# linum-uqam/ViT-OCM-WMSegmentation

Hardware: AMD Instinct MI355X
Metric: OCM tiles/s (224x224, ViT-S/16 attention-map inference) (higher is better)
Workload: dtype bf16x3

## Files before the change

vit-ocm-wmsegmentation_amd/csrc/gemm_core.h:

```cpp
#pragma once
#include <type_traits>
#include "common.h"

#ifdef OCM_GEMM_STAMPS
__device__ unsigned long long g_wstamps[512 * 16 * 8];
#define WSTAMP(k)                                                                                       \
    do {                                                                                                \
        if (t == nsteps / 2 && (threadIdx.x & 63) == 0 && blockIdx.x < 512)                              \
            g_wstamps[(blockIdx.x * 16 + (threadIdx.x >> 6 & 15)) * 8 + (k)] = __builtin_readcyclecounter(); \
    } while (0)
__device__ unsigned long long g_stamps[8192 * 8];
#define STAMP(i)                                                                                        \
    do {                                                                                                \
        if (threadIdx.x == 0 && blockIdx.x < 8192) g_stamps[blockIdx.x * 8 + (i)] = __builtin_readcyclecounter(); \
    } while (0)
#else
#define STAMP(i) ((void)0)
#define WSTAMP(k) ((void)0)
#endif

template <int BM_, int BN_, int WAVES_M_, int WAVES_N_, int MF16_ = 0>
struct GemmCfg {
    static constexpr int BM = BM_, BN = BN_, WAVES_M = WAVES_M_, WAVES_N = WAVES_N_, MF16 = MF16_;
    static constexpr int NT = WAVES_M * WAVES_N * OCM_WAVE;
// ... 187 lines not shown
    for (int i = 0; i < A_CH; ++i) {
        const int q = tid + NT * i, row = q >> 3;
        a_h[i] = al.row(min(m0 + row, M - 1));
        a_off[i] = lds_off(row, cc);
    }
#pragma unroll
    for (int i = 0; i < B_CH; ++i) {
        const int q = tid + NT * i, row = q >> 3;
        b_h[i] = (const char *)W + (int64_t)min(n0 + row, N - 1) * ldw * (int)sizeof(E) + cc * 16;
        b_off[i] = lds_off(row, cc);
    }
    struct Slot {
        typename ALoad::Raw a[A_CH];
        Chunk b[B_CH];
    };
    auto issue = [&](Slot &sl, int t) {
#pragma unroll
        for (int i = 0; i < A_CH; ++i) sl.a[i] = al.load(a_h[i], t, cc);
#pragma unroll
#if defined(OCM_ABL) && (OCM_ABL == 9 || OCM_ABL == 10)
        for (int i = 0; i < B_CH; ++i) sl.b[i] = *(const Chunk *)(b_h[i]);
#else
        for (int i = 0; i < B_CH; ++i) {
            if constexpr (aload_w_tail<ALoad>::v) {
                sl.b[i] = Chunk{};
                if (t * 128 + cc * 16 < al.w_row_bytes) sl.b[i] = *(const Chunk *)(b_h[i] + t * 128);
            } else {
                sl.b[i] = *(const Chunk *)(b_h[i] + t * 128);
            }
        }
#endif
    };
    auto commit = [&](int buf, const Slot &sl) {
#pragma unroll
        for (int i = 0; i < A_CH; ++i) *(Chunk *)(As + buf * BM * 128 + a_off[i]) = ALoad::finish(sl.a[i], cc);
#pragma unroll
        for (int i = 0; i < B_CH; ++i) *(Chunk *)(Bs + buf * BN * 128 + b_off[i]) = sl.b[i];
    };
    auto compute = [&](int buf) {
        mma_step<Cfg, E, SWAP>(As + buf * BM * 128 + (wm * 32) * 128, Bs + buf * BN * 128 + (wn * 32) * 128, r, h, acc);
    };

    constexpr int ACCL = accl_of<Cfg, E>();
#pragma unroll
    for (int j = 0; j < TN; ++j) {
        const int nb = n0 + (j * Cfg::WAVES_N + wn) * 32;
#pragma unroll
        for (int e = 0; e < 16; ++e) {
            const float bv = bias ? bias[min(nb + (SWAP ? acc_rpos<ACCL>(e, lane) : acc_cpos<ACCL>(e, lane)), N - 1)] : 0.f;
#pragma unroll
            for (int i = 0; i < TM; ++i) acc[i][j][e] = bv;
        }
    }

    if constexpr (KSTEPS > 0) {
#if defined(OCM_ABL) && OCM_ABL == 11
        auto issue2 = [&](Slot &sl, int t) { if (t < 3) issue(sl, min(t, KSTEPS - 1)); };
#else
        auto issue2 = [&](Slot &sl, int t) { issue(sl, min(t, KSTEPS - 1)); };
#endif
        Slot s0, s1;
        issue2(s0, 0);
        issue2(s1, 1);
        commit(0, s0);
        issue2(s0, 2);
        lds_barrier();
#ifdef OCM_GEMM_STAMPS
        STAMP(6);
#endif
        if constexpr (KSTEPS % 2 == 0 && Elem<E>::MODE == 2 && NT == 512 && OCM_PINGPONG) {
            auto phase_barrier = [&]() {
                __builtin_amdgcn_sched_barrier(0);
                lds_barrier();
                __builtin_amdgcn_sched_barrier(0);
            };
            const int grp = __builtin_amdgcn_readfirstlane(wave >> 2);
            if (grp == 0) {
                for (int t = 0; t < KSTEPS; t += 2) {
                    compute(0);
                    phase_barrier();
                    commit(1, s1);
                    issue2(s1, t + 3);
                    phase_barrier();
                    compute(1);
                    phase_barrier();
                    commit(0, s0);
                    issue2(s0, t + 4);
                    phase_barrier();
                }
            } else {
                for (int t = 0; t < KSTEPS; t += 2) {
                    commit(1, s1);
                    issue2(s1, t + 3);
                    phase_barrier();
                    compute(0);
                    phase_barrier();
                    commit(0, s0);
                    issue2(s0, t + 4);
                    phase_barrier();
                    compute(1);
                    phase_barrier();
                }
            }
        } else if constexpr (KSTEPS % 2 == 0) {
            for (int t = 0; t < KSTEPS; t += 2) {
                compute(0);
                commit(1, s1);
                issue2(s1, t + 3);
                lds_barrier();
                compute(1);
                commit(0, s0);
                issue2(s0, t + 4);
                lds_barrier();
            }
        } else {
#pragma unroll
            for (int t = 0; t < KSTEPS; ++t) {
                compute(t & 1);
                if (t & 1) {
                    if (t + 1 < KSTEPS) commit(0, s0);
                    issue2(s0, t + 3);
                } else {
                    if (t + 1 < KSTEPS) commit(1, s1);
                    issue2(s1, t + 3);
                }
                lds_barrier();
            }
        }
    } else {
        const int nt = K / KROW;
        Slot s0;
        issue(s0, 0);
        commit(0, s0);
        lds_barrier();
        for (int t = 0; t < nt; ++t) {
            const int buf = t & 1;
            if (t + 1 < nt) issue(s0, t + 1);
            compute(buf);
            if (t + 1 < nt) commit(buf ^ 1, s0);
            lds_barrier();
        }
    }
}

#define OCM_VMCNT(n) asm volatile("s_waitcnt vmcnt(%0)" ::"n"(n) : "memory")

__device__ __forceinline__ void raw_barrier() {
    asm volatile("s_waitcnt lgkmcnt(0)" ::: "memory");
    __builtin_amdgcn_s_barrier();
    asm volatile("" ::: "memory");
}

template <int LPS, int S>
__device__ __forceinline__ void wait_vm_steps(int younger) {
    if constexpr (S == 0) {
        OCM_VMCNT(0);
    } else {
        if (younger >= S)
            OCM_VMCNT(S * LPS);
        else
            wait_vm_steps<LPS, S - 1>(younger);
    }
}

template <int CNT, int NW, int AUX = 0>
__device__ __forceinline__ void dma_rows(__amdgpu_buffer_rsrc_t rs, char *img, const int (&voff)[CNT], int wave,
                                         int soff) {
#if defined(__HIP_DEVICE_COMPILE__)
    typedef __attribute__((address_space(3))) void *lds_ptr;
#pragma unroll
    for (int j = 0; j < CNT; ++j)
        __builtin_amdgcn_raw_ptr_buffer_load_lds(rs, (lds_ptr)(img + (j * NW + wave) * 1024), 16, voff[j], soff, 0, AUX);
#endif
}

template <int CNT, int AUX = 0>
__device__ __forceinline__ void dma_pieces(__amdgpu_buffer_rsrc_t rs, char *img, const int (&voff)[CNT], const int (&piece)[CNT],
                                           int soff) {
#if defined(__HIP_DEVICE_COMPILE__)
    typedef __attribute__((address_space(3))) void *lds_ptr;
#pragma unroll
    for (int j = 0; j < CNT; ++j)
        __builtin_amdgcn_raw_ptr_buffer_load_lds(rs, (lds_ptr)(img + piece[j] * 1024), 16, voff[j], soff, 0, AUX);
#endif
}

template <class Cfg, class E, bool SWAP, int KSTEPS, int NSTAGE, int A_AUX = 0>
__device__ __forceinline__ void gemm_mainloop_dma(const E *__restrict__ A, int64_t lda, const E *__restrict__ W,
                                                  int64_t ldw, int m0, int n0, int M, int N, int K, char *smem,
                                                  f32x16 (&acc)[Cfg::TM][Cfg::TN], const float *__restrict__ bias) {
    constexpr int BM = Cfg::BM, BN = Cfg::BN, NT = Cfg::NT, NW = NT / 64;
    constexpr int TM = Cfg::TM, TN = Cfg::TN;
    constexpr int A_P = BM / 8, A_I = (A_P + NW - 1) / NW, B_I = BN / 8 / NW, LPS = A_I + B_I;
    constexpr int STAGE = (BM + BN) * 128, D = NSTAGE - 1;
    static_assert(BM % 8 == 0 && BN % (8 * NW) == 0 && (A_P % NW == 0 || 2 * (A_P % NW) >= NW), "each wave fills whole groups of 8 rows");
    static_assert(NSTAGE >= 2 && NSTAGE <= 4, "2..4 LDS stages");
    const int tid = threadIdx.x, lane = tid & 63;
    const int wave = __builtin_amdgcn_readfirstlane(tid >> 6);
    const int wm = wave / Cfg::WAVES_N, wn = wave % Cfg::WAVES_N;
    const int r = lane & 31, h = lane >> 5;
    const int esz = (int)sizeof(E);
    const int nsteps = KSTEPS > 0 ? KSTEPS : K / Elem<E>::KROW;

    auto bound = [](int64_t rows, int64_t ld_bytes) {
        const int64_t b = rows * ld_bytes;
        return (unsigned)(b > 0xFFFFFFFFll ? 0xFFFFFFFFll : b);
    };
    const auto rsA = __builtin_amdgcn_make_buffer_rsrc((void *)((const char *)A + (int64_t)m0 * lda * esz), 0,
                                                       bound(M - m0, lda * esz), 0x00020000);
    const auto rsB = __builtin_amdgcn_make_buffer_rsrc((void *)((const char *)W + (int64_t)n0 * ldw * esz), 0,
                                                       bound(N - n0, ldw * esz), 0x00020000);
    int voffA[A_I], voffB[B_I];
    int pieceA[A_I];
#pragma unroll
    for (int j = 0; j < A_I; ++j) {
        int pc = j * NW + wave;
        if (pc >= A_P) pc -= A_P % NW;
        pieceA[j] = pc;
        const int rho = pc * 8 + (lane >> 3);
        voffA[j] = rho * (int)(lda * esz) + (((lane & 7) ^ ((rho >> 1) & 7)) << 4);
    }
#pragma unroll
    for (int j = 0; j < B_I; ++j) {
        const int rho = (j * NW + wave) * 8 + (lane >> 3);
        voffB[j] = rho * (int)(ldw * esz) + (((lane & 7) ^ ((rho >> 1) & 7)) << 4);
    }
#define OCM_DMA_ISSUE(t, buf)                                                   \
    do {                                                                        \
        char *st_ = smem + (buf) * STAGE;                                       \
        dma_pieces<A_I, A_AUX>(rsA, st_, voffA, pieceA, (t) * 128);             \
        dma_rows<B_I, NW>(rsB, st_ + BM * 128, voffB, wave, (t) * 128);         \
    } while (0)
    auto compute = [&](int buf) {
        const char *st = smem + buf * STAGE;
        mma_step<Cfg, E, SWAP>(st + (wm * 32) * 128, st + BM * 128 + (wn * 32) * 128, r, h, acc, wm);
    };

    constexpr int ACCL = accl_of<Cfg, E>();
    constexpr int NBV = SWAP ? 16 : (ACCL ? 2 : 1);
    float bv[TN][NBV];
#pragma unroll
    for (int j = 0; j < TN; ++j) {
        const int nb = n0 + (j * Cfg::WAVES_N + wn) * 32;
#pragma unroll
        for (int e = 0; e < NBV; ++e)
            bv[j][e] = bias ? bias[min(nb + (SWAP ? acc_rpos<ACCL>(e, lane) : acc_cpos<ACCL>(4 * e, lane)), N - 1)] : 0.f;
    }
#pragma unroll
    for (int t = 0; t < D; ++t)
        if (t < nsteps) OCM_DMA_ISSUE(t, t);
#pragma unroll
    for (int j = 0; j < TN; ++j)
#pragma unroll
        for (int i = 0; i < TM; ++i)
#pragma unroll
            for (int e = 0; e < 16; ++e) acc[i][j][e] = bv[j][SWAP ? e : (ACCL ? ((e >> 2) & 1) : 0)];
    int bc = 0, bi = D % NSTAGE;
#ifdef OCM_GEMM_STAMPS
    unsigned long long stamp_wait = 0;
#endif
    for (int t = 0; t < nsteps; ++t) {
        const int younger = min(D - 1, nsteps - 1 - t);
#ifdef OCM_GEMM_STAMPS
        const unsigned long long tw0 = __builtin_readcyclecounter();
#endif
        WSTAMP(0);
        wait_vm_steps<LPS, NSTAGE - 2>(younger);
        WSTAMP(1);
#ifdef OCM_GEMM_STAMPS
        const unsigned long long tw1 = __builtin_readcyclecounter();
#endif
        raw_barrier();
#ifdef OCM_GEMM_STAMPS
        if (t == 0) STAMP(6);
        if (t > 0) {
            const unsigned long long tw2 = __builtin_readcyclecounter();
            stamp_wait += ((tw2 - tw1) << 32) | ((tw1 - tw0) & 0xFFFFFFFFull);
        }
#endif
        WSTAMP(2);
#if !defined(OCM_ABL) || OCM_ABL != 2
        if (t + D < nsteps) OCM_DMA_ISSUE(t + D, bi);
#endif
        __builtin_amdgcn_sched_barrier(0);
        WSTAMP(3);
        compute(bc);
#ifdef OCM_GEMM_STAMPS
        if (t == nsteps / 2) {
            __builtin_amdgcn_sched_barrier(0);
            asm volatile("v_mov_b32 %0, %0\n\ts_nop 0" : "+v"(acc[TM - 1][TN - 1][15]));
            WSTAMP(4);
        }
#endif
        bc = bc + 1 == NSTAGE ? 0 : bc + 1;
        bi = bi + 1 == NSTAGE ? 0 : bi + 1;
    }
    raw_barrier();
#ifdef OCM_GEMM_STAMPS
    if (threadIdx.x == 0 && blockIdx.x < 8192) g_stamps[blockIdx.x * 8 + 7] = stamp_wait;
#endif
#undef OCM_DMA_ISSUE
}

constexpr int EPI_MAXS = 6;
struct EpiPre {
    f32x2 raw[EPI_MAXS];
    f32x2 cd;
};
struct EpiNoPre {};
template <class Cfg, class Epi>
__device__ __forceinline__ auto epi_prefetch(const Epi &epi, int m0, int n0, int M, int N) {
    if constexpr (Epi::ROWTAB) {
        EpiPre p;
#pragma unroll
        for (int i = 0; i < EPI_MAXS; ++i) p.raw[i] = f32x2{0.f, 0.f};
        p.cd = f32x2{0.f, 0.f};
        if (threadIdx.x < Cfg::BM) epi.row_raw(min(m0 + (int)threadIdx.x, M - 1), p.raw);
        if (threadIdx.x < Cfg::BN) p.cd = epi.col_entry(min(n0 + (int)threadIdx.x, N - 1));
        return p;
    } else {
        return EpiNoPre();
    }
}

template <class Cfg, bool SWAP, class Epi, int LDS_AVAIL = Cfg::LDS_BYTES, class Pre = EpiNoPre, int ACCL = 0>
__device__ __forceinline__ void run_epilogue(const f32x16 (&acc)[Cfg::TM][Cfg::TN], char *smem, const Epi &epi, int m0,
                                             int n0, bool active = true, const Pre *pre = nullptr) {
    f32x2 *rowtab = (f32x2 *)(smem + LDS_AVAIL), *coltab = rowtab + Cfg::BM;
    if constexpr (Epi::ROWTAB) {
        if (threadIdx.x < Cfg::BM) rowtab[threadIdx.x] = epi.row_final(pre->raw);
        if (threadIdx.x < Cfg::BN) coltab[threadIdx.x] = pre->cd;
    }
    const int lane = threadIdx.x & 63, wave = threadIdx.x >> 6;
    const int wm = wave / Cfg::WAVES_N, wn = wave % Cfg::WAVES_N;
    const int r = lane & 31, h = lane >> 5;
    if constexpr (Cfg::BM * Cfg::BN * 4 <= LDS_AVAIL) {
        constexpr int COLS = SWAP ? Cfg::BM : Cfg::BN;
        float *C = (float *)smem;
        if (active)
#pragma unroll
        for (int i = 0; i < Cfg::TM; ++i)
#pragma unroll
            for (int j = 0; j < Cfg::TN; ++j) {
                const bool half = Cfg::HALF && i == Cfg::TM - 1;
                const int tm = half ? (Cfg::TM - 1) * Cfg::RB + wm * 16 : (i * Cfg::WAVES_M + wm) * 32, tn = (j * Cfg::WAVES_N + wn) * 32;
                const int row0 = SWAP ? tn : tm, col0 = SWAP ? tm : tn;
#pragma unroll
                for (int e = 0; e < (half ? 8 : 16); ++e)
                    C[(row0 + acc_rpos<ACCL>(e, lane)) * COLS + col0 + acc_cpos<ACCL>(e, lane)] = acc[i][j][e];
            }
        STAMP(2);
        lds_barrier();
        STAMP(3);
        if (active) epi.template run<PassCfg<Cfg::BM, Cfg::BN, Cfg::NT>>((const float *)C, m0, n0, rowtab, coltab);
    } else if constexpr (!SWAP) {
        constexpr int PASS = Cfg::RB * Cfg::BN * 4;
        static_assert(PASS <= LDS_AVAIL, "a row band must fit the operand LDS");
        constexpr int NBUF = 2 * PASS <= LDS_AVAIL ? 2 : 1;
#pragma unroll
        for (int i = 0; i < Cfg::TM; ++i) {
            if (NBUF == 1 && i) lds_barrier();
            float *C = (float *)(smem + (i % NBUF) * PASS);
            const bool half = Cfg::HALF && i == Cfg::TM - 1;
            if (active)
#pragma unroll
            for (int j = 0; j < Cfg::TN; ++j) {
                const int col0 = (j * Cfg::WAVES_N + wn) * 32;
#pragma unroll
                for (int e = 0; e < (half ? 8 : 16); ++e)
                    C[(wm * (half ? 16 : 32) + acc_rpos<ACCL>(e, lane)) * Cfg::BN + col0 + acc_cpos<ACCL>(e, lane)] = acc[i][j][e];
            }
            lds_barrier();
            if (active) {
                if (half)
                    epi.template run<PassCfg<Cfg::RB / 2, Cfg::BN, Cfg::NT>>((const float *)C, m0 + i * Cfg::RB, n0, rowtab + i * Cfg::RB, coltab);
                else
                    epi.template run<PassCfg<Cfg::RB, Cfg::BN, Cfg::NT>>((const float *)C, m0 + i * Cfg::RB, n0, rowtab + i * Cfg::RB, coltab);
            }
        }
    } else {
        static_assert(!Cfg::HALF, "half tiles: normal orientation only");
        constexpr int PASS = Cfg::CB * Cfg::BM * 4;
        static_assert(PASS <= LDS_AVAIL, "a column band must fit the operand LDS");
        constexpr int NBUF = 2 * PASS <= LDS_AVAIL ? 2 : 1;
#pragma unroll
        for (int j = 0; j < Cfg::TN; ++j) {
            if (NBUF == 1 && j) lds_barrier();
            float *C = (float *)(smem + (j % NBUF) * PASS);
            if (active)
#pragma unroll
            for (int i = 0; i < Cfg::TM; ++i) {
                const int col0 = (i * Cfg::WAVES_M + wm) * 32;
#pragma unroll
                for (int e = 0; e < 16; ++e)
                    C[(wn * 32 + acc_rpos<ACCL>(e, lane)) * Cfg::BM + col0 + acc_cpos<ACCL>(e, lane)] = acc[i][j][e];
            }
            lds_barrier();
            if (active) epi.template run<PassCfg<Cfg::BM, Cfg::CB, Cfg::NT>>((const float *)C, m0, n0 + j * Cfg::CB, rowtab, coltab + j * Cfg::CB);
        }
    }
}

template <class Cfg, class E, bool SWAP, int KSTEPS, int NSTAGE, class Epi, int A_AUX = 0>
__global__ __launch_bounds__(Cfg::NT) void gemm_dma_kernel(const E *__restrict__ A, int64_t lda, const E *__restrict__ W,
                                                           int64_t ldw, int M, int N, int K, Epi epi) {
    extern __shared__ __attribute__((aligned(16))) char smem[];
    const int tiles_n = (N + Cfg::BN - 1) / Cfg::BN;
    const int id = xcd_remap(blockIdx.x, gridDim.x);
    const int tm = id / tiles_n, tn = id - tm * tiles_n;
    const int m0 = tm * Cfg::BM, n0 = tn * Cfg::BN;
    f32x16 acc[Cfg::TM][Cfg::TN];
    const auto pre = epi_prefetch<Cfg>(epi, m0, n0, M, N);
    STAMP(0);
#if defined(OCM_ABL) && OCM_ABL == 4
#pragma unroll
    for (int i = 0; i < Cfg::TM; ++i)
#pragma unroll
        for (int j = 0; j < Cfg::TN; ++j)
#pragma unroll
            for (int e = 0; e < 16; ++e) acc[i][j][e] = (float)(threadIdx.x + e);
#else
    gemm_mainloop_dma<Cfg, E, SWAP, KSTEPS, NSTAGE, A_AUX>(A, lda, W, ldw, m0, n0, M, N, K, smem, acc, epi.bias);
#endif
    STAMP(1);
#if defined(OCM_ABL) && OCM_ABL == 3
#pragma unroll
    for (int i = 0; i < Cfg::TM; ++i)
#pragma unroll
        for (int j = 0; j < Cfg::TN; ++j) asm volatile("" ::"v"(acc[i][j]));
#else
    run_epilogue<Cfg, SWAP, Epi, NSTAGE * (Cfg::BM + Cfg::BN) * 128, decltype(pre), accl_of<Cfg, E>()>(acc, smem, epi, m0, n0, true, &pre);
#endif
    STAMP(4);
#ifdef OCM_GEMM_STAMPS
    __builtin_amdgcn_s_waitcnt(0);
    STAMP(5);
#endif
}

template <class Cfg, class E, bool SWAP, int KSTEPS, class ALoad, class Epi>
__global__ __launch_bounds__(Cfg::NT) void gemm_kernel(ALoad al, const E *__restrict__ W, int64_t ldw, int M, int N,
                                                       int K, Epi epi) {
    extern __shared__ __attribute__((aligned(16))) char smem[];
    const int tiles_n = (N + Cfg::BN - 1) / Cfg::BN;
    const int id = xcd_remap(blockIdx.x, gridDim.x);
    const int tm = id / tiles_n, tn = id - tm * tiles_n;
    const int m0 = tm * Cfg::BM, n0 = tn * Cfg::BN;
    f32x16 acc[Cfg::TM][Cfg::TN];
    const auto pre = epi_prefetch<Cfg>(epi, m0, n0, M, N);
    STAMP(0);
    gemm_mainloop<Cfg, E, SWAP, KSTEPS>(al, W, ldw, m0, n0, M, N, K, smem, acc, epi.bias);
    STAMP(1);
    run_epilogue<Cfg, SWAP, Epi, Cfg::LDS_BYTES, decltype(pre), accl_of<Cfg, E>()>(acc, smem, epi, m0, n0, true, &pre);
    STAMP(4);
#ifdef OCM_GEMM_STAMPS
    __builtin_amdgcn_s_waitcnt(0);
    STAMP(5);
#endif
}
```

vit-ocm-wmsegmentation_amd/csrc/gemm_kernels.h:

```cpp
#pragma once
#include <type_traits>
#include "gemm_core.h"
#include "launch.h"
#include "dev_knobs.h"

int ocm_wt_mask();

#ifndef OCM_SMALLM_STAGES
#define OCM_SMALLM_STAGES 4
#endif
constexpr int OCM_SMALLM_ROWS = 4096;
typedef GemmCfg<128, 128, 2, 2> Cfg128x128;
typedef GemmCfg<128, 128, 2, 4> Cfg128x128q;
typedef GemmCfg<128, 128, 2, 4, 1> Cfg128x128q16;
typedef GemmCfg<128, 128, 2, 2, 1> Cfg128x128m16;
typedef GemmCfg<160, 128, 2, 4, 1> Cfg160x128q16;
typedef GemmCfg<256, 256, 2, 4, 1> Cfg256x256m16;
typedef GemmCfg<64, 128, 2, 2> Cfg64x128;
typedef GemmCfg<64, 128, 2, 4> Cfg64x128w;
typedef GemmCfg<64, 64, 2, 2> Cfg64x64;
typedef GemmCfg<256, 256, 2, 4> Cfg256x256;

static inline bool big_tiles_pay(int M, int N, int K) {
    return K >= 768 && N % 256 == 0 && (long)((M + 255) / 256) * (N / 256) >= 512;
// ... 746 lines not shown
                                const float v = e < 4 ? v0[e & 3] : v1[e & 3];
                                store_act1((E *)nullptr, (char *)vt + ((int64_t)(bb * H + head) * hd + d) * npad * 4, tt, v);
                                if (qkv32) qkv32[((((int64_t)2 * B + bb) * H + head) * ntok + tt) * hd + d] = v;
                            }
                            if (++tt == ntok) {
                                tt = 0;
                                ++bb;
                            }
                        }
                    }
                }
                return;
            }
        }
        constexpr int RS = NT >= BM ? NT / BM : 1;
        static_assert(NT >= BM, "one lane per token column");
        if (threadIdx.x >= RS * BM) return;
        const int col = threadIdx.x % BM, m = m0 + col;
        if (m >= M) return;
        const int b = m / ntok, t = m - b * ntok;
        const f32x2 mr = rowtab[col];
        const float mu = mr[0], rstd = mr[1];
#pragma unroll 4
        for (int row = threadIdx.x / BM; row < BN; row += RS) {
            const int rem = rem0 + row;
            const int head = hd == 64 ? rem >> 6 : rem / hd, d = rem - head * hd;
            float v = C[row * BM + col];
            if (ln.stats) {
                const f32x2 cd = coltab[row];
                v = fmaf(rstd, fmaf(-mu, cd[0], v), cd[1]);
            }
            if (vt) store_act1((E *)nullptr, (char *)vt + ((int64_t)(b * H + head) * hd + d) * npad * (int)sizeof(E), t, v);
            if (qkv32) qkv32[((((int64_t)2 * B + b) * H + head) * ntok + t) * hd + d] = v;
        }
    }
};

template <class Cfg, class E, int KSTEPS>
__global__ __launch_bounds__(Cfg::NT) void qkv_kernel(RowLoader<E> al, const E *__restrict__ W, int M, int D,
                                                      EpiQK<E> eqk, EpiVt<E> ev) {
    extern __shared__ __attribute__((aligned(16))) char smem[];
    const int N = 3 * D, K = D;
    const int tiles_n = (ev.want_v ? N : 2 * D) / Cfg::BN;
    const int id = xcd_remap(blockIdx.x, gridDim.x);
    const int tm = id / tiles_n, tn = id - tm * tiles_n;
    const int m0 = tm * Cfg::BM, n0 = tn * Cfg::BN;
    f32x16 acc[Cfg::TM][Cfg::TN];
    const auto pre = epi_prefetch<Cfg>(eqk, m0, n0, M, N);
    if (n0 < 2 * D) {
        gemm_mainloop<Cfg, E, false, KSTEPS>(al, W, K, m0, n0, M, N, K, smem, acc, eqk.bias);
        run_epilogue<Cfg, false, EpiQK<E>, Cfg::LDS_BYTES, decltype(pre), accl_of<Cfg, E>()>(acc, smem, eqk, m0, n0, true, &pre);
    } else {
        gemm_mainloop<Cfg, E, true, KSTEPS>(al, W, K, m0, n0, M, N, K, smem, acc, ev.bias);
        run_epilogue<Cfg, true, EpiVt<E>, Cfg::LDS_BYTES, decltype(pre), accl_of<Cfg, E>()>(acc, smem, ev, m0, n0, true, &pre);
    }
}

template <class Cfg, class E, int KSTEPS, int NSTAGE>
__global__ __launch_bounds__(Cfg::NT) void qkv_dma_kernel(const E *__restrict__ A, const E *__restrict__ W, int M, int D,
                                                          EpiQK<E> eqk, EpiVt<E> ev) {
    extern __shared__ __attribute__((aligned(16))) char smem[];
    const int N = 3 * D, K = D;
    const int tiles_n = (ev.want_v ? N : 2 * D) / Cfg::BN;
    const int id = xcd_remap(blockIdx.x, gridDim.x);
    const int tm = id / tiles_n, tn = id - tm * tiles_n;
    const int m0 = tm * Cfg::BM, n0 = tn * Cfg::BN;
    f32x16 acc[Cfg::TM][Cfg::TN];
    const auto pre = epi_prefetch<Cfg>(eqk, m0, n0, M, N);
    constexpr int RING = NSTAGE * (Cfg::BM + Cfg::BN) * 128;
    if (n0 < 2 * D) {
        gemm_mainloop_dma<Cfg, E, false, KSTEPS, NSTAGE>(A, K, W, K, m0, n0, M, N, K, smem, acc, eqk.bias);
        run_epilogue<Cfg, false, EpiQK<E>, RING, decltype(pre), accl_of<Cfg, E>()>(acc, smem, eqk, m0, n0, true, &pre);
    } else {
        gemm_mainloop_dma<Cfg, E, true, KSTEPS, NSTAGE>(A, K, W, K, m0, n0, M, N, K, smem, acc, ev.bias);
        run_epilogue<Cfg, true, EpiVt<E>, RING, decltype(pre), accl_of<Cfg, E>()>(acc, smem, ev, m0, n0, true, &pre);
    }
}

template <class Cfg, class E, int KSTEPS, int NSTAGE>
static hipError_t launch_qkv_dma_ks(const E *a, const E *w, int M, int D, const EpiQK<E> &eqk, const EpiVt<E> &ev,
                                    hipStream_t s) {
    auto kern = qkv_dma_kernel<Cfg, E, KSTEPS, NSTAGE>;
    constexpr int LDS = NSTAGE * (Cfg::BM + Cfg::BN) * 128 + (Cfg::BM + Cfg::BN) * 8;
    static OptinMask optin;
    if (hipError_t e = lds_optin((const void *)kern, LDS, optin); e != hipSuccess) return e;
    const int tiles = ((M + Cfg::BM - 1) / Cfg::BM) * ((ev.want_v ? 3 : 2) * D / Cfg::BN);
    kern<<<dim3(tiles), dim3(Cfg::NT), LDS, s>>>(a, w, M, D, eqk, ev);
    return hipGetLastError();
}

template <class Cfg, class E, int NSTAGE>
static hipError_t launch_qkv_dma(const E *a, const E *w, int M, int D, const EpiQK<E> &eqk, const EpiVt<E> &ev,
                                 hipStream_t s) {
    switch (D / Elem<E>::KROW) {
        case 12: return launch_qkv_dma_ks<Cfg, E, 12, NSTAGE>(a, w, M, D, eqk, ev, s);
        case 24: return launch_qkv_dma_ks<Cfg, E, 24, NSTAGE>(a, w, M, D, eqk, ev, s);
        default: break;
    }
    return launch_qkv_dma_ks<Cfg, E, 0, NSTAGE>(a, w, M, D, eqk, ev, s);
}

template <class Cfg, class E, int KSTEPS>
static hipError_t launch_qkv_ks(const RowLoader<E> &al, const E *w, int M, int D, const EpiQK<E> &eqk,
                                const EpiVt<E> &ev, hipStream_t s) {
    auto kern = qkv_kernel<Cfg, E, KSTEPS>;
    constexpr int LDS = Cfg::LDS_BYTES + (Cfg::BM + Cfg::BN) * 8;
    static OptinMask optin;
    if (hipError_t e = lds_optin((const void *)kern, LDS, optin); e != hipSuccess) return e;
    const int tiles = ((M + Cfg::BM - 1) / Cfg::BM) * ((ev.want_v ? 3 : 2) * D / Cfg::BN);
    kern<<<dim3(tiles), dim3(Cfg::NT), LDS, s>>>(al, w, M, D, eqk, ev);
    return hipGetLastError();
}

template <class Cfg, class E>
static hipError_t launch_qkv_cfg(const RowLoader<E> &al, const E *w, int M, int D, const EpiQK<E> &eqk,
                                 const EpiVt<E> &ev, hipStream_t s) {
    switch (D / Elem<E>::KROW) {
        case 6: return launch_qkv_ks<Cfg, E, 6>(al, w, M, D, eqk, ev, s);
        case 12: return launch_qkv_ks<Cfg, E, 12>(al, w, M, D, eqk, ev, s);
        case 24: return launch_qkv_ks<Cfg, E, 24>(al, w, M, D, eqk, ev, s);
        default: break;
    }
    return launch_qkv_ks<Cfg, E, 0>(al, w, M, D, eqk, ev, s);
}

template <class E>
hipError_t launch_qkv_e(const E *a, const E *w, const float *bias, E *q, E *k, E *vt, float *qkv_f32, int batch,
                               int n_tokens, int n_pad, int heads, int head_dim, bool want_v, hipStream_t s,
                               const LnFold &ln) {
    const int D = heads * head_dim, M = batch * n_tokens;
    if (head_dim != 64 && head_dim != 128 && (q || k || vt)) return hipErrorInvalidValue;
    if (head_dim % 8) return hipErrorInvalidValue;
    if (D % 64) return hipErrorInvalidValue;
    RowLoader<E> al{a, D};
    EpiQK<E> eqk{bias, q, k, qkv_f32, M, n_tokens, n_pad, heads, D, batch, head_dim};
    eqk.wt = (ocm_wt_mask() >> 1) & 1;
    EpiVt<E> ev{bias, vt, qkv_f32, M, n_tokens, n_pad, heads, D, batch, head_dim, want_v};
    if (ln.stats) {
        eqk.ln = ev.ln = ln;
        eqk.bias = ev.bias = nullptr;
        if (OCM_KNOB(6) == 1) eqk.ln.stats = ev.ln.stats = nullptr;
        if (OCM_KNOB(6) == 2) eqk.ln.nslot = ev.ln.nslot = 1;
    }
    if constexpr (Elem<E>::MODE == 0)
        if (D % 256 == 0 && big_tiles_pay(M, 3 * D, D)) return launch_qkv_cfg<Cfg256x256, E>(al, w, M, D, eqk, ev, s);
    const long t128 = (long)((M + 127) / 128) * (3 * D / 128);
    if constexpr (Elem<E>::MODE == 2) {
        if (D % 128 == 0 && M > 64) {
#ifdef OCM_DEV
            switch (OCM_KNOB(3)) {
                case 1: return launch_qkv_dma<Cfg128x128, E, 2>(a, w, M, D, eqk, ev, s);
                case 2: return launch_qkv_dma<Cfg128x128q, E, 2>(a, w, M, D, eqk, ev, s);
                case 3: return launch_qkv_dma<Cfg64x128, E, 2>(a, w, M, D, eqk, ev, s);
                case 4: if (D % 256 == 0) return launch_qkv_dma<Cfg256x256, E, 2>(a, w, M, D, eqk, ev, s); break;
                case 5: return launch_qkv_dma<Cfg128x128q16, E, 2>(a, w, M, D, eqk, ev, s);
                case 6: if (D % 256 == 0) return launch_qkv_dma<Cfg256x256m16, E, 2>(a, w, M, D, eqk, ev, s); break;
                default: break;
            }
#endif
            if (OCM_KNOB(3) == 0) {
                if (M <= OCM_SMALLM_ROWS) return launch_qkv_dma<Cfg64x128w, E, OCM_SMALLM_STAGES>(a, w, M, D, eqk, ev, s);
                if (D % 256 == 0 && big_tiles_pay(M, 3 * D, D)) return launch_qkv_dma<Cfg256x256m16, E, 2>(a, w, M, D, eqk, ev, s);
                if (t128 >= 512) return launch_qkv_dma<Cfg128x128q16, E, 2>(a, w, M, D, eqk, ev, s);
            }
        }
    }
    if (D % 128 == 0 && t128 >= 512) return launch_qkv_cfg<Cfg128x128q, E>(al, w, M, D, eqk, ev, s);
    if (D % 128 == 0) return launch_qkv_cfg<Cfg64x128, E>(al, w, M, D, eqk, ev, s);
    return launch_qkv_cfg<Cfg64x64, E>(al, w, M, D, eqk, ev, s);
}

template <class E>
__device__ __forceinline__ int gather_k_of(int t, int cc) {
    constexpr int MODE = Elem<E>::MODE;
    return MODE == 0 ? t * 64 + cc * 8 : MODE == 1 ? t * 32 + cc * 4 : t * 32 + (cc & 3) * 8;
}
struct GatherRaw {
    f32x4 lo, hi;
};
template <class E>
__device__ __forceinline__ typename Elem<E>::Chunk gather_finish(const GatherRaw &r, int cc) {
    if constexpr (Elem<E>::MODE == 0) {
        return cvt8(r.lo, r.hi);
    } else if constexpr (Elem<E>::MODE == 1) {
        return r.lo;
    } else {
        bf16x8 hi, lo;
        split8(r.lo, r.hi, hi, lo);
        const bf16x8 sel = cc < 4 ? hi : lo;
        return __builtin_bit_cast(f32x4, sel);
    }
}

template <class E>
struct PatchLoader {
    const float *image;
    int64_t sb, sc, sy;
    const int32_t *origins;
    int P, wp, p, pp;
    typedef const float *Handle;
    typedef GatherRaw Raw;
    __device__ __forceinline__ Handle row(int m) const {
        const int b = m / P, pi = m - b * P;
        const int py = pi / wp, px = pi - py * wp;
        int y0 = 0, x0 = 0;
        if (origins) {
            y0 = origins[2 * b];
            x0 = origins[2 * b + 1];
        }
        return image + (int64_t)b * sb + (int64_t)(y0 + py * p) * sy + x0 + px * p;
    }
    __device__ __forceinline__ Raw load(Handle h, int t, int cc) const {
        constexpr int MODE = Elem<E>::MODE;
        const int k = gather_k_of<E>(t, cc);
        const int c = k / pp, rem = k - c * pp;
        const int dy = rem / p, dx = rem - dy * p;
        const float *ptr = h + (int64_t)c * sc + (int64_t)dy * sy + dx;
        Raw r;
        r.lo = *(const f32x4 *)ptr;
        r.hi = r.lo;
        if (MODE != 1) r.hi = *(const f32x4 *)(ptr + 4);
        return r;
    }
    __device__ __forceinline__ static typename Elem<E>::Chunk finish(const Raw &r, int cc) { return gather_finish<E>(r, cc); }
};

struct EpiPatch {
    static constexpr bool ROWTAB = false;
    const float *bias, *pos;
    float *x;
    int M, P, ntok, D;
    const float *mask, *mask_tok;
    StatsOut so;
    template <class Cfg>
    __device__ __forceinline__ void run(const float *C, int m0, int n0, const f32x2 *, const f32x2 *) const {
        constexpr int BM = Cfg::BM, BN = Cfg::BN, NT = Cfg::NT, CPR = BN / 4;
        if (so.stats) return run_stats<Cfg>(C, m0, n0);
#pragma unroll 4
        for (int q = threadIdx.x; q < BM * CPR; q += NT) {
            const int row = q / CPR, col = (q - row * CPR) * 4;
            const int m = m0 + row, n = n0 + col;
            if (m >= M || n >= D) continue;
            const int b = m / P, t = m - b * P;
            f32x4 v = *(const f32x4 *)(C + row * BN + col);
            if (mask) {
                const float w = mask[m], omw = 1.0f - w;
                const f32x4 tk = *(const f32x4 *)(mask_tok + n);
#pragma unroll
                for (int e = 0; e < 4; ++e) v[e] = v[e] * omw + tk[e] * w;
            }
            v += *(const f32x4 *)(pos + (int64_t)(1 + t) * D + n);
            *(f32x4 *)(x + ((int64_t)b * ntok + 1 + t) * D + n) = v;
        }
    }
    template <class Cfg>
    __device__ __forceinline__ void run_stats(const float *C, int m0, int n0) const {
        constexpr int BM = Cfg::BM, BN = Cfg::BN, NT = Cfg::NT, CPR = BN / 4;
        static_assert((BM * CPR) % NT == 0 && CPR <= 32 && (CPR & (CPR - 1)) == 0, "CPR lanes of one wave half own a row");
        const int sl = threadIdx.x & (CPR - 1), col = sl * 4, n = n0 + col;
        const bool nok = n < D;
        const int nc = min(n, D - 4);
#pragma unroll 1
        for (int row = threadIdx.x / CPR; row < BM; row += NT / CPR) {
            const int m = m0 + row;
            const bool ok = nok && m < M;
            const int mc = min(m, M - 1);
            const int b = mc / P, t = mc - b * P;
            f32x4 v = *(const f32x4 *)(C + row * BN + col);
            if (mask) {
                const float w = mask[mc], omw = 1.0f - w;
                const f32x4 tk = *(const f32x4 *)(mask_tok + nc);
#pragma unroll
                for (int e = 0; e < 4; ++e) v[e] = v[e] * omw + tk[e] * w;
            }
            v += *(const f32x4 *)(pos + (int64_t)(1 + t) * D + nc);
            const int64_t xrow = (int64_t)b * ntok + 1 + t;
            const float sh = so.tok_shift ? so.tok_shift[1 + t] : 0.f;
            float s1 = 0.f, s2 = 0.f;
            if (ok) {
                *(f32x4 *)(x + xrow * D + n) = v;
                if (so.shift && n0 == 0 && sl == 0) so.shift[xrow] = sh;
                v -= sh;
                bf16x4 hi, lo;
                split4(v, hi, lo);
                char *g = (char *)so.xs + xrow * D * 4 + sp_off(n);
                *(bf16x4 *)g = hi;
                *(bf16x4 *)(g + 64) = lo;
                s1 = (v[0] + v[1]) + (v[2] + v[3]);
                s2 = fmaf(v[0], v[0], fmaf(v[1], v[1], fmaf(v[2], v[2], v[3] * v[3])));
            }
#pragma unroll
            for (int o = CPR / 2; o > 0; o >>= 1) {
                s1 += __shfl_xor(s1, o, 64);
                s2 += __shfl_xor(s2, o, 64);
            }
            if (m < M && sl < BN / 64 && n0 + 64 * sl < D) {
                const f32x2 val = {sl ? 0.f : s1, sl ? 0.f : s2};
                *((f32x2 *)so.stats + xrow * (D >> 6) + (n0 >> 6) + sl) = val;
            }
        }
    }
};

template <class E>
hipError_t launch_patch_e(const PatchArgs &pa, const E *w, const float *bias, const float *pos, float *x, int dim,
                                 hipStream_t s, const StatsOut &so) {
    const int P = pa.hp * pa.wp, M = pa.batch * P, K = pa.chans * pa.p * pa.p;
    PatchLoader<E> al{pa.image, pa.sb, pa.sc, pa.sy, pa.origins, P, pa.wp, pa.p, pa.p * pa.p};
    EpiPatch epi{bias, pos, x, M, P, P + 1, dim, pa.mask, pa.mask_tok, so};
    if constexpr (Elem<E>::MODE == 2)
        if (dim % 128 == 0 && M > 64 && M <= 1024) return launch_gemm<Cfg64x128w, E, false>(al, w, K, M, dim, K, epi, s);
    if (dim % 128 == 0 && M > 64) return launch_gemm<Cfg64x128, E, false>(al, w, K, M, dim, K, epi, s);
    return launch_gemm<Cfg64x64, E, false>(al, w, K, M, dim, K, epi, s);
}
```

Baseline: 27530.

## Add double-buffered gather+DMA GEMM path for large-batch patch embedding

Adds a new GEMM mainloop for the patch-embedding layer. The image-patch A operand is gathered through registers one step ahead while the weight B tile is streamed into LDS with buffer DMA, using a two-stage LDS ring. It also specializes the K step count at compile time and uses 128x128 tiles with 8 waves. The path is taken when M exceeds 1024 and is meant to overlap the irregular patch gather with the MMA work. The patch embed is a small share of ViT-S inference, and the larger tiles may reduce occupancy.

```diff
diff --git a/vit-ocm-wmsegmentation_amd/csrc/gemm_core.h b/vit-ocm-wmsegmentation_amd/csrc/gemm_core.h
--- a/vit-ocm-wmsegmentation_amd/csrc/gemm_core.h
+++ b/vit-ocm-wmsegmentation_amd/csrc/gemm_core.h
@@ -513,6 +513,98 @@
 #undef OCM_DMA_ISSUE
 }
 
+template <class Cfg, class E, int KSTEPS, class ALoad>
+__device__ __forceinline__ void gemm_mainloop_dma_gather(const ALoad &al, const E *__restrict__ W, int64_t ldw, int m0,
+                                                         int n0, int M, int N, int K, char *smem,
+                                                         f32x16 (&acc)[Cfg::TM][Cfg::TN], const float *__restrict__ bias) {
+    typedef typename Elem<E>::Chunk Chunk;
+    static_assert(Elem<E>::MODE == 2 && !Cfg::HALF, "split-bf16 operands, whole 32-row tiles");
+    constexpr int BM = Cfg::BM, BN = Cfg::BN, NT = Cfg::NT, NW = NT / 64;
+    constexpr int TM = Cfg::TM, TN = Cfg::TN, A_CH = Cfg::A_CH;
+    constexpr int B_I = BN / 8 / NW, GL = 2 * A_CH;
+    constexpr int STAGE = (BM + BN) * 128;
+    static_assert(BN % (8 * NW) == 0, "each wave fills whole groups of 8 W rows");
+    const int tid = threadIdx.x, lane = tid & 63;
+    const int wave = __builtin_amdgcn_readfirstlane(tid >> 6);
+    const int wm = wave / Cfg::WAVES_N, wn = wave % Cfg::WAVES_N;
+    const int r = lane & 31, h = lane >> 5;
+    const int esz = (int)sizeof(E);
+    const int nsteps = KSTEPS > 0 ? KSTEPS : K / Elem<E>::KROW;
+
+    const int64_t wbytes = (int64_t)(N - n0) * ldw * esz;
+    const auto rsB = __builtin_amdgcn_make_buffer_rsrc((void *)((const char *)W + (int64_t)n0 * ldw * esz), 0,
+                                                       (unsigned)(wbytes > 0xFFFFFFFFll ? 0xFFFFFFFFll : wbytes), 0x00020000);
+    int voffB[B_I];
+#pragma unroll
+    for (int j = 0; j < B_I; ++j) {
+        const int rho = (j * NW + wave) * 8 + (lane >> 3);
+        voffB[j] = rho * (int)(ldw * esz) + (((lane & 7) ^ ((rho >> 1) & 7)) << 4);
+    }
+    const int cc = tid & 7;
+    typename ALoad::Handle a_h[A_CH];
+    int a_off[A_CH];
+#pragma unroll
+    for (int i = 0; i < A_CH; ++i) {
+        const int row = (tid + NT * i) >> 3;
+        a_h[i] = al.row(min(m0 + row, M - 1));
+        a_off[i] = lds_off(row, cc);
+    }
+    typename ALoad::Raw slot[A_CH];
+    auto pin = [&]() {
+        asm volatile("" ::: "memory");
+        __builtin_amdgcn_sched_barrier(0);
+    };
+    auto gather = [&](int t) {
+#pragma unroll
+        for (int i = 0; i < A_CH; ++i) slot[i] = al.load(a_h[i], t, cc);
+    };
+    auto commit = [&](int buf) {
+#pragma unroll
+        for (int i = 0; i < A_CH; ++i) *(Chunk *)(smem + buf * STAGE + a_off[i]) = ALoad::finish(slot[i], cc);
+    };
+    auto dma_w = [&](int t, int buf) { dma_rows<B_I, NW>(rsB, smem + buf * STAGE + BM * 128, voffB, wave, t * 128); };
+
+    float bv[TN];
+#pragma unroll
+    for (int j = 0; j < TN; ++j)
+        bv[j] = bias ? bias[min(n0 + (j * Cfg::WAVES_N + wn) * 32 + acc_cpos<0>(0, lane), N - 1)] : 0.f;
+    gather(0);
+    pin();
+    commit(0);
+    pin();
+    dma_w(0, 0);
+    pin();
+    if (nsteps > 1) gather(1);
+    pin();
+#pragma unroll
+    for (int j = 0; j < TN; ++j)
+#pragma unroll
+        for (int i = 0; i < TM; ++i)
+#pragma unroll
+            for (int e = 0; e < 16; ++e) acc[i][j][e] = bv[j];
+    for (int t = 0; t < nsteps; ++t) {
+        const int buf = t & 1;
+        pin();
+        if (t + 1 < nsteps)
+            OCM_VMCNT(GL);
+        else
+            OCM_VMCNT(0);
+        raw_barrier();
+        pin();
+        if (t + 1 < nsteps) {
+            commit(buf ^ 1);
+            pin();
+            dma_w(t + 1, buf ^ 1);
+            pin();
+            if (t + 2 < nsteps) gather(t + 2);
+            pin();
+        }
+        const char *st = smem + buf * STAGE;
+        mma_step<Cfg, E, false>(st + (wm * 32) * 128, st + BM * 128 + (wn * 32) * 128, r, h, acc, wm);
+    }
+    raw_barrier();
+}
+
 constexpr int EPI_MAXS = 6;
 struct EpiPre {
     f32x2 raw[EPI_MAXS];
diff --git a/vit-ocm-wmsegmentation_amd/csrc/gemm_kernels.h b/vit-ocm-wmsegmentation_amd/csrc/gemm_kernels.h
--- a/vit-ocm-wmsegmentation_amd/csrc/gemm_kernels.h
+++ b/vit-ocm-wmsegmentation_amd/csrc/gemm_kernels.h
@@ -1072,6 +1072,46 @@
     }
 };
 
+template <class Cfg, class E, int KSTEPS, class ALoad, class Epi>
+__global__ __launch_bounds__(Cfg::NT) void gemm_dma_gather_kernel(ALoad al, const E *__restrict__ W, int64_t ldw, int M,
+                                                                  int N, int K, Epi epi) {
+    extern __shared__ __attribute__((aligned(16))) char smem[];
+    const int tiles_n = (N + Cfg::BN - 1) / Cfg::BN;
+    const int id = xcd_remap(blockIdx.x, gridDim.x);
+    const int tm = id / tiles_n, tn = id - tm * tiles_n;
+    const int m0 = tm * Cfg::BM, n0 = tn * Cfg::BN;
+    f32x16 acc[Cfg::TM][Cfg::TN];
+    const auto pre = epi_prefetch<Cfg>(epi, m0, n0, M, N);
+    gemm_mainloop_dma_gather<Cfg, E, KSTEPS>(al, W, ldw, m0, n0, M, N, K, smem, acc, epi.bias);
+    run_epilogue<Cfg, false, Epi, 2 * (Cfg::BM + Cfg::BN) * 128, decltype(pre), accl_of<Cfg, E>()>(acc, smem, epi, m0, n0, true, &pre);
+}
+
+template <class Cfg, class E, int KSTEPS, class ALoad, class Epi>
+static hipError_t launch_gemm_dma_gather_ks(const ALoad &al, const E *w, int64_t ldw, int M, int N, int K, const Epi &epi,
+                                            hipStream_t s) {
+    static_assert(!Epi::ROWTAB, "no epilogue tables behind the ring");
+    constexpr int LDS = 2 * (Cfg::BM + Cfg::BN) * 128;
+    static_assert(LDS <= 80 * 1024, "two workgroups per CU");
+    auto kern = gemm_dma_gather_kernel<Cfg, E, KSTEPS, ALoad, Epi>;
+    static OptinMask optin;
+    if (hipError_t e = lds_optin((const void *)kern, LDS, optin); e != hipSuccess) return e;
+    const int tiles = ((M + Cfg::BM - 1) / Cfg::BM) * (N / Cfg::BN);
+    kern<<<dim3(tiles), dim3(Cfg::NT), LDS, s>>>(al, w, ldw, M, N, K, epi);
+    return hipGetLastError();
+}
+
+template <class Cfg, class E, class ALoad, class Epi>
+static hipError_t launch_gemm_dma_gather(const ALoad &al, const E *w, int64_t ldw, int M, int N, int K, const Epi &epi,
+                                         hipStream_t s) {
+    if (K % Elem<E>::KROW || N % Cfg::BN) return hipErrorInvalidValue;
+    switch (K / Elem<E>::KROW) {
+        case 6: return launch_gemm_dma_gather_ks<Cfg, E, 6>(al, w, ldw, M, N, K, epi, s);
+        case 24: return launch_gemm_dma_gather_ks<Cfg, E, 24>(al, w, ldw, M, N, K, epi, s);
+        default: break;
+    }
+    return launch_gemm_dma_gather_ks<Cfg, E, 0>(al, w, ldw, M, N, K, epi, s);
+}
+
 template <class E>
 hipError_t launch_patch_e(const PatchArgs &pa, const E *w, const float *bias, const float *pos, float *x, int dim,
                                  hipStream_t s, const StatsOut &so) {
@@ -1079,6 +1119,9 @@
     PatchLoader<E> al{pa.image, pa.sb, pa.sc, pa.sy, pa.origins, P, pa.wp, pa.p, pa.p * pa.p};
     EpiPatch epi{bias, pos, x, M, P, P + 1, dim, pa.mask, pa.mask_tok, so};
     if constexpr (Elem<E>::MODE == 2)
+        if (dim % 128 == 0 && K % 32 == 0 && M > 1024 && OCM_KNOB(4) != 3)
+            return launch_gemm_dma_gather<Cfg128x128q, E>(al, w, K, M, dim, K, epi, s);
+    if constexpr (Elem<E>::MODE == 2)
         if (dim % 128 == 0 && M > 64 && M <= 1024) return launch_gemm<Cfg64x128w, E, false>(al, w, K, M, dim, K, epi, s);
     if (dim % 128 == 0 && M > 64) return launch_gemm<Cfg64x128, E, false>(al, w, K, M, dim, K, epi, s);
     return launch_gemm<Cfg64x64, E, false>(al, w, K, M, dim, K, epi, s);
```

Result: no change. 27430 (-0.4%).
